# shao-lab/MotifScan

Measured on AMD Instinct MI355X. Metric: scanned bp*motifs per second (region_bp x n_motifs), both strands, p=1e-4 cutoffs, higher is better.
Workload: dtype f64 (every hit decision and score, as in the reference) behind an fp6 x fp4 one-hot matrix-core pre-filter (exact f32 accumulate)

## Files before the change

### motifscan_amd/csrc/ms_order.hip

```cpp
#include <algorithm>

#include "ms_device.h"

namespace ms {

namespace {

constexpr int kOrderThreads = 256;
constexpr int kOrderTile = 1024;
constexpr int kOrderExt = 256;
constexpr int kOrderWin = kOrderTile + kOrderExt;
constexpr int kOverflowBlocks = 256;

struct OrderRun {
    int64_t start;
    uint64_t prev;
};

struct OrderOut {
    int64_t *seq_idx;
    int64_t *pos;
    int8_t *strand;
    double *score;
    int64_t *motif_first;
    unsigned long long *region_counts;
    int rbits, pbits;
    int32_t P;
};

__device__ __forceinline__ bool decode_hit(const OrderOut &O, int64_t g, int64_t n, uint64_t k, double v, bool has_prev, uint64_t pk,
                                           uint32_t *motif_out) {
    const int ms = O.rbits + O.pbits + 1;
    const uint64_t pair = k >> (O.pbits + 1);
    const uint32_t motif = (uint32_t) (k >> ms);
    O.seq_idx[g] = (int64_t) (pair & ((1ULL << O.rbits) - 1ULL));
    O.pos[g] = (int64_t) ((k >> 1) & ((1ULL << O.pbits) - 1ULL));
    O.strand[g] = (int8_t) ((k & 1ULL) ? 2 : 1);
    O.score[g] = v;
    const uint32_t pm = has_prev ? (uint32_t) (pk >> ms) : 0u;
    if (!has_prev || pm != motif)
        for (int64_t q = has_prev ? (int64_t) pm + 1 : 0; q <= (int64_t) motif; q++) O.motif_first[q] = g;
    if (g == n - 1)
        for (int64_t q = (int64_t) motif + 1; q <= O.P; q++) O.motif_first[q] = n;
    *motif_out = motif;
    return !has_prev || (pk >> (O.pbits + 1)) != pair;
}

constexpr int kOrderMotifSlots = 8;
__device__ __forceinline__ void count_pairs(unsigned long long *region_counts, bool new_pair, uint32_t motif, unsigned int *lds, uint32_t m_base) {
    unsigned long long todo = __ballot(new_pair);
    while (todo) {
        const int leader = __ffsll((long long) todo) - 1;
        const uint32_t m = __shfl(motif, leader);
        const unsigned long long same = __ballot(new_pair && motif == m);
        if ((int) (threadIdx.x & 63) == leader) {
            if (lds && m - m_base < (uint32_t) kOrderMotifSlots) atomicAdd(&lds[m - m_base], (unsigned int) __popcll(same));
            else atomicAdd(&region_counts[m], (unsigned long long) __popcll(same));
        }
        todo &= ~same;
    }
}

__global__ void __launch_bounds__(kOrderThreads) order_finalize_kernel(const uint64_t *__restrict__ keys, int64_t n, const unsigned long long *__restrict__ n_dev,
                                                                      int L, int run_cap, OrderOut O, OrderRun *__restrict__ ovf,
                                                                      unsigned long long *__restrict__ ovf_n, uint64_t ovf_cap) {
    constexpr int kPer = kOrderWin / kOrderThreads, kSegs = kOrderWin / 64;
    __shared__ uint64_t K[kOrderWin];
    __shared__ uint64_t S[kOrderWin];
    __shared__ double V[kOrderWin];
    __shared__ uint8_t D[kOrderWin];
    __shared__ int seg_first[kSegs], seg_last[kSegs];
    __shared__ unsigned int rc[kOrderMotifSlots];
    if (n_dev) { const unsigned long long nd = *n_dev; if ((unsigned long long) n > nd) n = (int64_t) nd; }
    const int64_t s0 = (int64_t) blockIdx.x * kOrderTile;
    if (s0 >= n) return;
    const int tid = (int) threadIdx.x, lane = tid & 63, w = tid >> 6;
    const int wn = (int) std::min<int64_t>(kOrderWin, n - s0);
    const int tn = std::min(kOrderTile, wn);
    uint64_t kr[kPer];
    double vr[kPer];
#pragma unroll
    for (int k = 0; k < kPer; k++) {
        const int i = tid + kOrderThreads * k;
        kr[k] = i < wn ? keys[s0 + i] : ~0ULL;
        vr[k] = i < wn ? O.score[s0 + i] : 0.0;
        K[i] = kr[k];
        D[i] = 0;
    }
    if (tid < kOrderMotifSlots) rc[tid] = 0;
    const uint64_t prevk = s0 > 0 ? keys[s0 - 1] : 0ULL;
    __syncthreads();
    unsigned long long msk[kPer];
#pragma unroll
    for (int k = 0; k < kPer; k++) {
        const int i = tid + kOrderThreads * k;
        const bool start = i < wn && (i == 0 ? (s0 == 0 || (prevk >> L) != (kr[k] >> L)) : (K[i - 1] >> L) != (kr[k] >> L));
        msk[k] = __ballot(start);
        if (lane == 0) {
            const int seg = w + (kOrderThreads / 64) * k;
            seg_first[seg] = msk[k] ? seg * 64 + __ffsll((long long) msk[k]) - 1 : kOrderWin;
            seg_last[seg] = msk[k] ? seg * 64 + 63 - __clzll((long long) msk[k]) : -1;
        }
    }
    __syncthreads();
    int lo = kOrderWin, hi = wn;
    for (int q = 0; q < kSegs; q++) lo = std::min(lo, seg_first[q]);
    if (tn == kOrderTile)
        for (int q = kOrderTile / 64; q < kSegs; q++) hi = std::min(hi, seg_first[q]);
    if (lo >= tn) return;
    const bool closed = hi < wn || s0 + wn == n;
    const int ms = O.rbits + O.pbits + 1;
    const uint32_t m_base = (uint32_t) (K[lo] >> ms);
    const unsigned long long le = lane == 63 ? ~0ULL : (2ULL << lane) - 1ULL;
#pragma unroll
    for (int k = 0; k < kPer; k++) {
        const int i = tid + kOrderThreads * k, seg = w + (kOrderThreads / 64) * k;
        if (i < lo || i >= hi) continue;
        int a = -1, b = wn;
        if (msk[k] & le) a = seg * 64 + 63 - __clzll((long long) (msk[k] & le));
        else for (int q = seg - 1; q >= 0 && a < 0; q--) a = seg_last[q];
        if (msk[k] & ~le) b = seg * 64 + __ffsll((long long) (msk[k] & ~le)) - 1;
        else for (int q = seg + 1; q < kSegs && b == wn; q++) b = std::min(wn, seg_first[q]);
        if ((b == hi && !closed) || b - a > run_cap) {
            if (i == a) {
                const unsigned long long e = atomicAdd(ovf_n, 1ULL);
                if (e < ovf_cap) ovf[e] = OrderRun{s0 + a, a > 0 ? K[a - 1] : prevk};
            }
            continue;
        }
        int rank = 0;
        for (int j = a; j < b; j++) rank += K[j] < kr[k] ? 1 : 0;
        S[a + rank] = kr[k];
        V[a + rank] = vr[k];
        D[a + rank] = 1;
    }
    __syncthreads();
#pragma unroll
    for (int k = 0; k < kPer; k++) {
        const int j = tid + kOrderThreads * k;
        bool new_pair = false;
        uint32_t motif = 0;
        if (j >= lo && j < hi && D[j]) {
            const bool run_start = (msk[k] >> lane) & 1ULL;
            const uint64_t pk = run_start ? (j == 0 ? prevk : K[j - 1]) : S[j - 1];
            new_pair = decode_hit(O, s0 + j, n, S[j], V[j], s0 + j > 0, pk, &motif);
        }
        count_pairs(O.region_counts, new_pair, motif, rc, m_base);
    }
    __syncthreads();
    if (tid < kOrderMotifSlots && rc[tid]) atomicAdd(&O.region_counts[m_base + tid], (unsigned long long) rc[tid]);
}

__global__ void __launch_bounds__(kOrderThreads) order_overflow_kernel(uint64_t *keys, uint64_t *tmp_keys, double *tmp_vals,
                                                                      int64_t n, const unsigned long long *__restrict__ n_dev, int L, OrderOut O,
                                                                      const OrderRun *__restrict__ ovf, const unsigned long long *__restrict__ ovf_n,
                                                                      uint64_t ovf_cap) {
    __shared__ uint32_t base[256];
    __shared__ uint32_t wcnt[kOrderThreads / 64][256];
    __shared__ int64_t s_end;
    if (n_dev) { const unsigned long long nd = *n_dev; if ((unsigned long long) n > nd) n = (int64_t) nd; }
    const unsigned long long cnt = std::min<unsigned long long>(*ovf_n, ovf_cap);
    const int tid = (int) threadIdx.x, lane = tid & 63, w = tid >> 6;
    const unsigned long long lt = (1ULL << lane) - 1ULL;
    for (unsigned long long e = blockIdx.x; e < cnt; e += gridDim.x) {
        const int64_t s = ovf[e].start;
        const uint64_t prev = ovf[e].prev;
        const uint64_t h = keys[s] >> L;
        if (tid == 0) s_end = n;
        __syncthreads();
        for (int64_t c = s + 1; c < n; c += kOrderThreads) {
            const int64_t j = c + tid;
            if (j < n && (keys[j] >> L) != h) atomicMin((unsigned long long *) &s_end, (unsigned long long) j);
            __syncthreads();
            if (s_end < n) break;
            __syncthreads();
        }
        const int64_t b = s_end;
        uint64_t *sk = keys, *dk = tmp_keys;
        double *sv = O.score, *dv = tmp_vals;
        for (int shift = 0; shift < L; shift += 8) {
            base[tid] = 0;
            for (int q = 0; q < kOrderThreads / 64; q++) wcnt[q][tid] = 0;
            __syncthreads();
            for (int64_t j = s + tid; j < b; j += kOrderThreads) atomicAdd(&base[(uint32_t) (sk[j] >> shift) & 255u], 1u);
            __syncthreads();
            if (tid == 0) {
                uint32_t acc = 0;
                for (int d = 0; d < 256; d++) { const uint32_t c = base[d]; base[d] = acc; acc += c; }
            }
            __syncthreads();
            for (int64_t c = s; c < b; c += kOrderThreads) {
                const int64_t j = c + tid;
                const bool live = j < b;
                const uint64_t k = live ? sk[j] : 0ULL;
                const double v = live ? sv[j] : 0.0;
                const uint32_t d = (uint32_t) (k >> shift) & 255u;
                unsigned long long peers = __ballot(live);
#pragma unroll
                for (int bit = 0; bit < 8; bit++) {
                    const unsigned long long m = __ballot((d >> bit) & 1u);
                    peers &= ((d >> bit) & 1u) ? m : ~m;
                }
                if (live && (peers >> lane) == 1ULL) wcnt[w][d] = (uint32_t) __popcll(peers);
                __syncthreads();
                if (live) {
                    uint32_t off = base[d] + (uint32_t) __popcll(peers & lt);
                    for (int q = 0; q < w; q++) off += wcnt[q][d];
                    dk[s + off] = k;
                    dv[s + off] = v;
                }
                __syncthreads();
                uint32_t add = 0;
                for (int q = 0; q < kOrderThreads / 64; q++) { add += wcnt[q][tid]; wcnt[q][tid] = 0; }
                base[tid] += add;
                __syncthreads();
            }
            uint64_t *tk = sk; sk = dk; dk = tk;
            double *tv = sv; sv = dv; dv = tv;
        }
        for (int64_t c = s; c < b; c += kOrderThreads) {
            const int64_t j = c + tid;
            bool new_pair = false;
            uint32_t motif = 0;
            if (j < b) new_pair = decode_hit(O, j, n, sk[j], sv[j], j > 0, j == s ? prev : sk[j - 1], &motif);
            count_pairs(O.region_counts, new_pair, motif, nullptr, 0);
        }
        __syncthreads();
    }
}

}

size_t order_overflow_bytes(size_t n, int run_cap) {
    const size_t min_len = (size_t) std::min(std::max(run_cap, 1), kOrderExt) + 1;
    return (n / min_len + 1) * sizeof(OrderRun);
}

int launch_order_finalize(uint64_t *keys, double *score, int64_t n, const unsigned long long *n_dev, int L, int rbits, int pbits, int32_t P,
                          int64_t *seq_idx, int64_t *pos, int8_t *strand, int64_t *motif_first, unsigned long long *region_counts,
                          uint64_t *tmp_keys, double *tmp_vals, void *ovf_buf, size_t ovf_bytes, unsigned long long *ovf_n, int run_cap,
                          hipStream_t st) {
    if (n == 0 || n_dev) {
        MS_HIP(hipMemsetAsync(motif_first, 0, ((size_t) P + 1) * sizeof(int64_t), st));
        if (n == 0) return MS_OK;
    }
    run_cap = std::max(run_cap, 1);
    OrderOut O;
    O.seq_idx = seq_idx; O.pos = pos; O.strand = strand; O.score = score; O.motif_first = motif_first; O.region_counts = region_counts;
    O.rbits = rbits; O.pbits = pbits; O.P = P;
    OrderRun *ovf = static_cast<OrderRun *>(ovf_buf);
    const uint64_t ovf_cap = ovf_bytes / sizeof(OrderRun);
    hipLaunchKernelGGL(order_finalize_kernel, dim3((unsigned) ((n + kOrderTile - 1) / kOrderTile)), dim3(kOrderThreads), 0, st, keys, n, n_dev,
                       L, run_cap, O, ovf, ovf_n, ovf_cap);
    MS_HIP(hipGetLastError());
    if (L < 63 && (1ULL << L) > (unsigned long long) std::min(run_cap, kOrderExt)) {
        hipLaunchKernelGGL(order_overflow_kernel, dim3(kOverflowBlocks), dim3(kOrderThreads), 0, st, keys, tmp_keys, tmp_vals, n, n_dev, L, O,
                           ovf, ovf_n, ovf_cap);
        MS_HIP(hipGetLastError());
    }
    return MS_OK;
}


__global__ void __launch_bounds__(256) fill_tail_kernel(uint64_t *__restrict__ keys, const unsigned long long *__restrict__ n_dev, uint64_t cap) {
    const unsigned long long n = *n_dev < cap ? *n_dev : cap;
    for (unsigned long long i = n + (unsigned long long) blockIdx.x * blockDim.x + threadIdx.x; i < cap; i += (unsigned long long) gridDim.x * blockDim.x)
        keys[i] = ~0ULL;
}

__global__ void __launch_bounds__(256) sort_fixup_kernel(uint64_t *__restrict__ keys, double *__restrict__ vals, int64_t n, const unsigned long long *__restrict__ n_dev) {
    if (n_dev) { const unsigned long long nd = *n_dev; if ((unsigned long long) n > nd) n = (int64_t) nd; }
    const int64_t i0 = ((int64_t) blockIdx.x * blockDim.x + threadIdx.x) * 4;
    if (i0 >= n) return;
    uint64_t k[4] = {0, 0, 0, 0};
    uint64_t hi[6];
    hi[0] = i0 > 0 ? keys[i0 - 1] >> kSortLowBits : ~0ULL;
    if (i0 + 4 <= n) {
        const ulonglong2 a = *reinterpret_cast<const ulonglong2 *>(keys + i0), b = *reinterpret_cast<const ulonglong2 *>(keys + i0 + 2);
        k[0] = a.x; k[1] = a.y; k[2] = b.x; k[3] = b.y;
    } else {
        for (int q = 0; q < 4; q++) k[q] = i0 + q < n ? keys[i0 + q] : ~0ULL;
    }
#pragma unroll
    for (int q = 0; q < 4; q++) hi[1 + q] = i0 + q < n ? k[q] >> kSortLowBits : ~0ULL;
    hi[5] = i0 + 4 < n ? keys[i0 + 4] >> kSortLowBits : ~0ULL;
#pragma unroll
    for (int q = 0; q < 4; q++) {
        const int64_t i = i0 + q;
        if (i + 1 >= n || hi[1 + q] == hi[q] || hi[1 + q] != hi[2 + q]) continue;
        if (q < 3 && hi[3 + q] != hi[1 + q]) {
            if (k[q] > k[q + 1]) {
                keys[i] = k[q + 1];
                keys[i + 1] = k[q];
                const double v0 = vals[i], v1 = vals[i + 1];
                vals[i] = v1;
                vals[i + 1] = v0;
            }
            continue;
        }
        const uint64_t h = hi[1 + q];
        int64_t len = 2;
        while (i + len < n && len < ((int64_t) 1 << kSortLowBits) && (keys[i + len] >> kSortLowBits) == h) len++;
        for (int64_t a = 1; a < len; a++) {
            const uint64_t ka = keys[i + a];
            const double va = vals[i + a];
            int64_t b = a;
            while (b > 0 && keys[i + b - 1] > ka) { keys[i + b] = keys[i + b - 1]; vals[i + b] = vals[i + b - 1]; b--; }
            keys[i + b] = ka;
            vals[i + b] = va;
        }
    }
}

int launch_sort_fixup(uint64_t *keys, double *vals, int64_t n, const unsigned long long *n_dev, hipStream_t st) {
    if (n == 0) return MS_OK;
    hipLaunchKernelGGL(sort_fixup_kernel, dim3((unsigned) ((n + 1023) / 1024)), dim3(256), 0, st, keys, vals, n, n_dev);
    MS_HIP(hipGetLastError());
    return MS_OK;
}

__global__ void __launch_bounds__(kOrderBuckets) bucket_plan_kernel(const BucketWeights bw, double mu, unsigned long long n_pred, unsigned long long need,
                                                                    unsigned long long cap_max, unsigned long long *__restrict__ tab) {
    __shared__ unsigned long long sum[kOrderBuckets];
    const int b = (int) threadIdx.x;
    const unsigned long long w = bw.w[b];
    unsigned long long cb = 0;
    if (w) {
        const double e = mu * (double) w / (double) bw.total;
        cb = (unsigned long long) ceil(e + 6.0 * __dsqrt_rn(e + 1.0)) + 1ULL;
        const unsigned long long extra = n_pred > need ? n_pred - need : 0ULL;
        cb += (unsigned long long) floor((double) extra * (double) w / (double) bw.total);
    }
    if (cb > cap_max) cb = cap_max;
    sum[b] = cb;
    __syncthreads();
    for (int d = 1; d < kOrderBuckets; d <<= 1) {
        const unsigned long long v = b >= d ? sum[b - d] : 0ULL;
        __syncthreads();
        sum[b] += v;
        __syncthreads();
    }
    const unsigned long long at = sum[b] - cb, base = at < n_pred ? at : n_pred;
    tab[b] = base;
    tab[kOrderBuckets + b] = cb < n_pred - base ? cb : n_pred - base;
    tab[2 * kOrderBuckets + b] = 0ULL;
    if (b == kOrderBuckets - 1) tab[3 * kOrderBuckets] = sum[b] < n_pred ? sum[b] : n_pred;
}

__global__ void __launch_bounds__(256) fill_tail_buckets_kernel(uint64_t *__restrict__ keys, const unsigned long long *__restrict__ tab, uint64_t n_pred,
                                                                unsigned long long *__restrict__ n_hits, unsigned long long *__restrict__ overflow) {
    const unsigned int b = blockIdx.y;
    unsigned long long lo, hi;
    if (b < (unsigned int) kOrderBuckets) {
        const unsigned long long base = tab[b], cap = tab[kOrderBuckets + b], fill = tab[2 * kOrderBuckets + b];
        lo = base + (fill < cap ? fill : cap);
        hi = base + cap;
        if (fill > cap && blockIdx.x == 0 && threadIdx.x == 0) *overflow = 1ULL;
    } else {
        lo = tab[3 * kOrderBuckets];
        hi = n_pred;
        if (blockIdx.x == 0) {
            __shared__ unsigned long long part[256];
            unsigned long long v = 0;
            for (int q = (int) threadIdx.x; q < kOrderBuckets; q += 256) {
                const unsigned long long cap = tab[kOrderBuckets + q], fill = tab[2 * kOrderBuckets + q];
                v += fill < cap ? fill : cap;
            }
            part[threadIdx.x] = v;
            __syncthreads();
            for (int d = 128; d > 0; d >>= 1) {
                if ((int) threadIdx.x < d) part[threadIdx.x] += part[threadIdx.x + d];
                __syncthreads();
            }
            if (threadIdx.x == 0) *n_hits = part[0];
        }
    }
    if (hi > n_pred) hi = n_pred;
    for (unsigned long long i = lo + (unsigned long long) blockIdx.x * blockDim.x + threadIdx.x; i < hi; i += (unsigned long long) gridDim.x * blockDim.x)
        keys[i] = ~0ULL;
}

int launch_bucket_plan(const BucketWeights &bw, double mu, unsigned long long n_pred, unsigned long long need, unsigned long long cap_max,
                       unsigned long long *tab, hipStream_t st) {
    hipLaunchKernelGGL(bucket_plan_kernel, dim3(1), dim3(kOrderBuckets), 0, st, bw, mu, n_pred, need, cap_max, tab);
    MS_HIP(hipGetLastError());
    return MS_OK;
}

int launch_fill_tail_buckets(uint64_t *keys, const unsigned long long *tab, uint64_t n_pred, unsigned long long *n_hits, unsigned long long *overflow,
                             hipStream_t st) {
    hipLaunchKernelGGL(fill_tail_buckets_kernel, dim3(16, kOrderBuckets + 1), dim3(256), 0, st, keys, tab, n_pred, n_hits, overflow);
    MS_HIP(hipGetLastError());
    return MS_OK;
}

int launch_fill_tail(uint64_t *keys, const unsigned long long *n_dev, uint64_t cap, hipStream_t st) {
    if (cap == 0) return MS_OK;
    hipLaunchKernelGGL(fill_tail_kernel, dim3(256), dim3(256), 0, st, keys, n_dev, cap);
    MS_HIP(hipGetLastError());
    return MS_OK;
}

__global__ void __launch_bounds__(256) finalize_kernel(const uint64_t *__restrict__ keys, int64_t n, const unsigned long long *__restrict__ n_dev,
                                                       int gbits, int32_t P, const DevSeq S,
                                                       int64_t *__restrict__ seq_idx, int64_t *__restrict__ pos,
// ... 128 lines not shown
```

### motifscan_amd/csrc/ms_fp64.hip

```cpp
#include "ms_device.h"

namespace ms {

__device__ __forceinline__ int64_t hit_coord(const HitOut &H, const DevSeq &S, int64_t r, int64_t g) {
    return H.pbits ? (int64_t) (((uint64_t) r << H.pbits) | (uint64_t) (g - S.offsets[r])) : g;
}

__device__ __forceinline__ void emit_hit(const HitOut &H, uint32_t motif, int64_t g, uint32_t sbit, double score) {
    const unsigned long long i = atomicAdd(H.n_hits, 1ULL);
    if (i < H.cap) {
        H.keys[i] = ((uint64_t) motif << (H.gbits + 1)) | ((uint64_t) g << 1) | sbit;
        H.vals[i] = score;
    }
}

__device__ __forceinline__ void test_and_emit(const HitOut &H, const DevPwm &Pw, uint32_t motif, int64_t g,
                                              double fwd, double rev, int strand_mask) {
    const double floor_ = Pw.raw_floor[motif];
    const bool try_f = (strand_mask & 1) && !(fwd < floor_);
    const bool try_r = (strand_mask & 2) && !(rev < floor_);
    if (!try_f && !try_r) return;
    const double max_raw = Pw.max_raw[motif];
    const double cutoff = Pw.cutoff[motif];
    const double s_f = try_f ? fwd / max_raw : 0.0, s_r = try_r ? rev / max_raw : 0.0;
// ... 89 lines not shown
    {
        const double2 *__restrict__ tab = Pw.tab2 + Pw.tab_off[p];
        for (int i = threadIdx.x; i < W * 4; i += 256) tab_lds[i] = tab[i];
        if (threadIdx.x == 0) tab_lds[W * 4] = make_double2(0.0, 0.0);
    }
    __syncthreads();
    const uint32_t zero = (uint32_t) W * 4u;
    for (int it = 0; it < kExactIter; it++) {
        const int64_t g = ((int64_t) blockIdx.x * kExactIter + it) * 256 + threadIdx.x;
        if (g >= S.n_bases) break;
        const int64_t r = find_region(S, g);
        if (g + W > S.offsets[r + 1]) continue;
        double fwd = 0.0, rev = 0.0;
        for (int c0 = 0; c0 < W; c0 += 32) {
            const uint64_t cw = code_window(S.codes, g + c0);
            const int n = (W - c0) < 32 ? (W - c0) : 32;
            const uint32_t skip = n_window(S.nmask, g + c0) | ~low_mask(n);
            for (int c1 = 0; c1 < n; c1 += 8) {
                double2 t[8];
#pragma unroll
                for (int k = 0; k < 8; k++) {
                    const int c = c1 + k;
                    const uint32_t idx = (uint32_t) (c0 + c) * 4u + ((uint32_t) (cw >> (2 * c)) & 3u);
                    t[k] = tab_lds[((skip >> c) & 1u) ? zero : idx];
                }
#pragma unroll
                for (int k = 0; k < 8; k++) { fwd += t[k].x; rev += t[k].y; }
            }
        }
        test_and_emit(H, Pw, (uint32_t) p, hit_coord(H, S, r, g), fwd, rev, strand_mask);
    }
}

constexpr int kRescoreU = 4;

__global__ void __launch_bounds__(256) rescore_kernel(const DevSeq S, const DevPwm Pw, const uint64_t *__restrict__ cand,
                                                      const unsigned long long *__restrict__ n_cand, uint64_t n_static, uint64_t cand_cap,
                                                      const FieldMeta *__restrict__ field_meta, int strand_mask,
                                                      const HitOut H) {
    __shared__ HitStage st;
    if (threadIdx.x == 0) st.n = 0;
    __syncthreads();
    unsigned long long n = n_static + *n_cand;
    if (n > cand_cap) n = cand_cap;
    constexpr int U = kRescoreU;
    const bool both = strand_mask == 3;
    const unsigned long long per_sub = (unsigned long long) gridDim.x * blockDim.x;
    const unsigned long long per_round = per_sub * U;
    const unsigned long long rounds = (n + per_round - 1) / per_round;
    const int4 *__restrict__ meta4 = reinterpret_cast<const int4 *>(field_meta);
    for (unsigned long long rd = 0; rd < rounds; rd++) {
        const unsigned long long i0 = rd * per_round + (unsigned long long) blockIdx.x * blockDim.x + threadIdx.x;
        uint64_t c[U];
        bool live[U];
#pragma unroll
        for (int u = 0; u < U; u++) {
            live[u] = i0 + u * per_sub < n;
            c[u] = live[u] ? cand[i0 + u * per_sub] : 0;
        }
        int64_t g[U];
        int4 bi[U];
        uint64_t cw[U];
        uint32_t nw[U], flags[U];
        int32_t group[U];
        int4 fm[U];
#pragma unroll
        for (int u = 0; u < U; u++) {
            g[u] = (int64_t) (c[u] >> 30);
            group[u] = (int32_t) ((c[u] >> 16) & 0x3FFFu);
            const uint32_t f = (uint32_t) c[u] & 0xFFFFu;
            flags[u] = both ? (f | (f >> 1)) & 0x5555u : f;
            bi[u] = S.blkinfo[g[u] >> 6];
            cw[u] = code_window(S.codes, g[u]);
            nw[u] = n_window(S.nmask, g[u]);
            fm[u] = flags[u] ? meta4[group[u] * kGroupFields + (__ffs((int) flags[u]) - 1)] : make_int4(-1, 0, 0, 0);
        }
        int64_t r[U], beg[U], end[U];
#pragma unroll
        for (int u = 0; u < U; u++) {
            const int64_t base = g[u] & ~(int64_t) 63;
            int64_t lo = bi[u].x, o0 = base + bi[u].y, o1 = base + bi[u].z, o2 = base + bi[u].w;
            if (bi[u].x < 0) {
                lo = S.blk2reg[g[u] >> 6];
                o0 = S.offsets[lo]; o1 = S.offsets[lo + 1];
                o2 = lo + 2 <= S.R ? S.offsets[lo + 2] : o1;
            }
            if (g[u] < o1) { r[u] = lo; beg[u] = o0; end[u] = o1; }
            else if (g[u] < o2) { r[u] = lo + 1; beg[u] = o1; end[u] = o2; }
            else { r[u] = find_region(S, g[u]); beg[u] = S.offsets[r[u]]; end[u] = S.offsets[r[u] + 1]; }
        }
#pragma unroll
        for (int u = 0; u < U; u++) {
            if (!live[u]) continue;
            const int64_t gk = H.pbits ? (int64_t) (((uint64_t) r[u] << H.pbits) | (uint64_t) (g[u] - beg[u])) : g[u];
            bool first = true;
            while (flags[u]) {
                const int field = __ffs((int) flags[u]) - 1;
                flags[u] &= flags[u] - 1u;
                int4 f4 = fm[u];
                if (!first) f4 = meta4[group[u] * kGroupFields + field];
                first = false;
                const int32_t m = f4.x;
                const int w = f4.y;
                if (m < 0) continue;
                if (g[u] + w > end[u]) continue;
                double fwd, rev;
                if (w <= 32 && Pw.tab32) score_window32(Pw.tab2, (uint32_t) f4.z, Pw.zero_bytes, w, cw[u], nw[u], fwd, rev);
                else score_window(S, Pw.tab2 + Pw.tab_off[m], w, g[u], fwd, rev);
                test_and_stage(st, H, Pw, (uint32_t) m, gk, fwd, rev, strand_mask, __int_as_float(f4.w));
            }
        }
        __syncthreads();
        const bool full = st.n > (unsigned int) (kHitStage - 256 * 2 * U);
        __syncthreads();
        if (full) stage_flush(st, H);
    }
    stage_flush(st, H);
}

int launch_exact_all(const DevSeq &S, const DevPwm &Pw, const int32_t *motifs, int32_t n_motifs, int strand_mask,
                     const HitOut &H, hipStream_t st, int max_width) {
    if (S.n_bases == 0 || n_motifs == 0) return MS_OK;
    const bool tiled = max_width >= 1 && max_width <= kExactTileMaxW && !measure_env("MS_EXACT_UNTILED");
    const size_t lds = tiled ? ((size_t) max_width * 4 + 1) * sizeof(double2) : 0;
    if (tiled && lds > 48 * 1024)
        MS_HIP(hipFuncSetAttribute(reinterpret_cast<const void *>(exact_tiled_kernel), hipFuncAttributeMaxDynamicSharedMemorySize, (int) lds));
    for (int32_t m0 = 0; m0 < n_motifs; m0 += 32768) {
        const int32_t n = n_motifs - m0 < 32768 ? n_motifs - m0 : 32768;
        if (tiled) {
            dim3 grid((unsigned) ((S.n_bases + 256 * kExactIter - 1) / (256 * kExactIter)), (unsigned) n);
            hipLaunchKernelGGL(exact_tiled_kernel, grid, dim3(256), lds, st, S, Pw, motifs + m0, strand_mask, H);
        } else {
            dim3 grid((unsigned) ((S.n_bases + 255) / 256), (unsigned) n);
            hipLaunchKernelGGL(exact_all_kernel, grid, dim3(256), 0, st, S, Pw, motifs + m0, strand_mask, H);
        }
        MS_HIP(hipGetLastError());
    }
    return MS_OK;
}

int launch_rescore(const DevSeq &S, const DevPwm &Pw, const uint64_t *cand, const unsigned long long *n_cand, uint64_t n_static,
                   uint64_t cand_cap, const FieldMeta *field_meta, int strand_mask, const HitOut &H, int n_blocks,
                   hipStream_t st) {
    hipLaunchKernelGGL(rescore_kernel, dim3((unsigned) n_blocks), dim3(256), 0, st, S, Pw, cand, n_cand, n_static, cand_cap,
                       field_meta, strand_mask, H);
    MS_HIP(hipGetLastError());
    return MS_OK;
}

constexpr int kRwThreads = 1024;
constexpr int kRwPerThread = 4;
constexpr int kRwChunk = kRwThreads * kRwPerThread;
constexpr int kRwBins = 4096;
typedef HitStageN<2048> RwStage;
struct RwStageBk : RwStage {
    unsigned int cnt[kOrderBuckets], room[kOrderBuckets];
    unsigned long long lo[kOrderBuckets];
};

__device__ __forceinline__ void stage_flush(RwStageBk &st, const BucketHitOut &H) {
    constexpr int kPer = RwStageBk::kCap / kRwThreads;
    static_assert(kPer * kRwThreads == RwStageBk::kCap && kOrderBuckets <= kRwThreads, "stage_flush: one pass of the block over the stage");
    __syncthreads();
    const unsigned int n = st.n < (unsigned int) RwStageBk::kCap ? st.n : (unsigned int) RwStageBk::kCap;
    if (threadIdx.x < (unsigned int) kOrderBuckets) st.cnt[threadIdx.x] = 0;
    __syncthreads();
    uint32_t bk[kPer], rank[kPer];
#pragma unroll
    for (int k = 0; k < kPer; k++) {
        const unsigned int i = threadIdx.x + (unsigned int) (k * kRwThreads);
        bk[k] = i < n ? (uint32_t) (st.keys[i] >> H.B.shift) & 255u : 0u;
        rank[k] = i < n ? atomicAdd(&st.cnt[bk[k]], 1u) : 0u;
    }
    __syncthreads();
    if (threadIdx.x < (unsigned int) kOrderBuckets && st.cnt[threadIdx.x] > 0) {
        const unsigned int b = threadIdx.x, c = st.cnt[b];
        const unsigned long long f = atomicAdd(&H.B.fill[b], (unsigned long long) c), cap = H.B.cap[b];
        const unsigned long long left = f < cap ? cap - f : 0ULL;
        st.lo[b] = H.B.base[b] + f;
        st.room[b] = left < (unsigned long long) c ? (unsigned int) left : c;
        if (left < (unsigned long long) c) *H.B.overflow = 1ULL;
    }
    __syncthreads();
#pragma unroll
    for (int k = 0; k < kPer; k++) {
        const unsigned int i = threadIdx.x + (unsigned int) (k * kRwThreads);
        if (i < n && rank[k] < st.room[bk[k]]) {
            const unsigned long long at = st.lo[bk[k]] + rank[k];
            if (at < H.cap) { H.keys[at] = st.keys[i]; H.vals[at] = st.vals[i]; }
        }
    }
    __syncthreads();
    if (threadIdx.x == 0) st.n = 0;
    __syncthreads();
}

template <class HO, class ST>
__global__ void __launch_bounds__(kRwThreads) rescore_carry_kernel(const DevSeq S, const DevPwm Pw, const uint64_t *__restrict__ cand,
                                                                   const unsigned long long *__restrict__ n_cand, uint64_t n_static, uint64_t cand_cap,
                                                                   const FieldMeta *__restrict__ field_meta, int strand_mask, const HO H) {
    extern __shared__ uint4 rw_lds4[];
    uint64_t *s_cw = reinterpret_cast<uint64_t *>(rw_lds4);
    uint64_t *s_gk = s_cw + kRwChunk;
    uint32_t *s_nw = reinterpret_cast<uint32_t *>(s_gk + kRwChunk);
    uint32_t *s_gf = s_nw + kRwChunk;
    uint32_t *bins = s_gf + kRwChunk;
    uint32_t *wave_tot = bins + kRwBins;
    ST &st = *reinterpret_cast<ST *>(wave_tot + 32);
    if (threadIdx.x == 0) st.n = 0;
    unsigned long long n = n_static + *n_cand;
    if (n > cand_cap) n = cand_cap;
    const bool both = strand_mask == 3;
    const int4 *__restrict__ meta4 = reinterpret_cast<const int4 *>(field_meta);
    const uint32_t lane = threadIdx.x & 63u, wave = threadIdx.x >> 6;
    const uint64_t pmask = H.pbits ? ((1ULL << H.pbits) - 1ULL) : 0ULL;
    const unsigned long long n_chunks = (n + kRwChunk - 1) / kRwChunk;
    for (unsigned long long ch = blockIdx.x; ch < n_chunks; ch += gridDim.x) {
        for (uint32_t i = threadIdx.x; i < (uint32_t) kRwBins; i += kRwThreads) bins[i] = 0;
        __syncthreads();
        {
            uint64_t cw[kRwPerThread], gk[kRwPerThread];
            uint32_t nw[kRwPerThread], gf[kRwPerThread], key[kRwPerThread], rank[kRwPerThread];
            int64_t g[kRwPerThread];
            int4 bi[kRwPerThread];
#pragma unroll
            for (int k = 0; k < kRwPerThread; k++) {
                const unsigned long long i = ch * kRwChunk + (unsigned long long) k * kRwThreads + threadIdx.x;
                const uint64_t rec = i < n ? cand[i] : 0ULL;
                g[k] = (int64_t) (rec >> 30);
                gf[k] = (uint32_t) rec & 0x3FFFFFFFu;
                if (!(gf[k] & 0xFFFFu)) { gf[k] = 0; g[k] = 0; }
                bi[k] = S.blkinfo[g[k] >> 6];
                cw[k] = code_window(S.codes, g[k]);
                nw[k] = n_window(S.nmask, g[k]);
            }
#pragma unroll
            for (int k = 0; k < kRwPerThread; k++) {
                const int64_t base = g[k] & ~(int64_t) 63;
                int64_t lo = bi[k].x, o0 = base + bi[k].y, o1 = base + bi[k].z, o2 = base + bi[k].w, r, beg, end;
                if (bi[k].x < 0) {
                    lo = S.blk2reg[g[k] >> 6];
                    o0 = S.offsets[lo]; o1 = S.offsets[lo + 1];
                    o2 = lo + 2 <= S.R ? S.offsets[lo + 2] : o1;
                }
                if (g[k] < o1) { r = lo; beg = o0; end = o1; }
                else if (g[k] < o2) { r = lo + 1; beg = o1; end = o2; }
                else { r = find_region(S, g[k]); beg = S.offsets[r]; end = S.offsets[r + 1]; }
                const uint64_t coord = H.pbits ? (((uint64_t) r << H.pbits) | (uint64_t) (g[k] - beg)) : (uint64_t) g[k];
                const int64_t room = end - g[k];
                gk[k] = (coord << 8) | (uint64_t) (room > 255 ? 255 : (room < 0 ? 0 : room));
                const uint32_t f = gf[k] & 0xFFFFu;
                const uint32_t fl = both ? (f | (f >> 1)) & 0x5555u : f;
                key[k] = fl ? (((gf[k] >> 16) << 4) | (uint32_t) (__ffs((int) fl) - 1)) & (uint32_t) (kRwBins - 1) : (uint32_t) (kRwBins - 1);
            }
#pragma unroll
            for (int k = 0; k < kRwPerThread; k++) rank[k] = atomicAdd(&bins[key[k]], 1u);
            __syncthreads();
            {
                const uint32_t b0 = bins[4 * threadIdx.x], b1 = bins[4 * threadIdx.x + 1], b2 = bins[4 * threadIdx.x + 2], b3 = bins[4 * threadIdx.x + 3];
                const uint32_t tot = b0 + b1 + b2 + b3;
                uint32_t v = tot;
#pragma unroll
                for (int d = 1; d < 64; d <<= 1) {
                    const uint32_t o = __shfl_up(v, d);
                    if ((int) lane >= d) v += o;
                }
                if (lane == 63u) wave_tot[wave] = v;
                __syncthreads();
                uint32_t base = 0;
                for (uint32_t w = 0; w < wave; w++) base += wave_tot[w];
                const uint32_t excl = base + v - tot;
                bins[4 * threadIdx.x] = excl;
                bins[4 * threadIdx.x + 1] = excl + b0;
                bins[4 * threadIdx.x + 2] = excl + b0 + b1;
                bins[4 * threadIdx.x + 3] = excl + b0 + b1 + b2;
            }
            __syncthreads();
#pragma unroll
            for (int k = 0; k < kRwPerThread; k++) {
                const uint32_t at = bins[key[k]] + rank[k];
                s_cw[at] = cw[k]; s_gk[at] = gk[k]; s_nw[at] = nw[k]; s_gf[at] = gf[k];
            }
        }
        __syncthreads();
        for (int round = 0; round < 2; round++) {
#pragma unroll
            for (int u = 0; u < 2; u++) {
                const uint32_t at = (uint32_t) (round * 2 + u) * kRwThreads + threadIdx.x;
                const uint32_t gfu = s_gf[at];
                const uint32_t f = gfu & 0xFFFFu;
                uint32_t flags = both ? (f | (f >> 1)) & 0x5555u : f;
                if (!flags) continue;
                const uint64_t cwu = s_cw[at], gku = s_gk[at];
                const uint32_t nwu = s_nw[at];
                const int32_t group = (int32_t) (gfu >> 16);
                const int room = (int) (gku & 0xFFu);
                const int64_t coord = (int64_t) (gku >> 8);
                while (flags) {
                    const int field = __ffs((int) flags) - 1;
                    flags &= flags - 1u;
                    const int4 f4 = meta4[group * kGroupFields + field];
                    const int32_t m = f4.x;
                    const int w = f4.y;
                    if (m < 0) continue;
                    if (w > room) continue;
                    double fwd, rev;
                    if (w <= 32 && Pw.tab32) score_window32(Pw.tab2, (uint32_t) f4.z, Pw.zero_bytes, w, cwu, nwu, fwd, rev);
                    else {
                        const int64_t gpos = H.pbits ? S.offsets[coord >> H.pbits] + (int64_t) ((uint64_t) coord & pmask) : coord;
                        score_window(S, Pw.tab2 + Pw.tab_off[m], w, gpos, fwd, rev);
                    }
                    test_and_stage(st, H, Pw, (uint32_t) m, coord, fwd, rev, strand_mask, __int_as_float(f4.w));
                }
            }
            stage_flush(st, H);
        }
    }
}

template <class ST>
static size_t rescore_carry_lds_bytes() { return (size_t) kRwChunk * 24 + (size_t) kRwBins * 4 + 32 * 4 + sizeof(ST) + 64; }
int rescore_carry_set_lds() {
    MS_HIP(hipFuncSetAttribute(reinterpret_cast<const void *>(rescore_carry_kernel<HitOut, RwStage>), hipFuncAttributeMaxDynamicSharedMemorySize,
                               (int) rescore_carry_lds_bytes<RwStage>()));
    MS_HIP(hipFuncSetAttribute(reinterpret_cast<const void *>(rescore_carry_kernel<BucketHitOut, RwStageBk>), hipFuncAttributeMaxDynamicSharedMemorySize,
                               (int) rescore_carry_lds_bytes<RwStageBk>()));
    return MS_OK;
}
int launch_rescore_carry(const DevSeq &S, const DevPwm &Pw, const uint64_t *cand, const unsigned long long *n_cand, uint64_t n_static,
                         uint64_t cand_cap, const FieldMeta *field_meta, int strand_mask, const HitOut &H, int n_blocks, hipStream_t st) {
    hipLaunchKernelGGL((rescore_carry_kernel<HitOut, RwStage>), dim3((unsigned) n_blocks), dim3(kRwThreads), rescore_carry_lds_bytes<RwStage>(), st, S, Pw,
                       cand, n_cand, n_static, cand_cap, field_meta, strand_mask, H);
    MS_HIP(hipGetLastError());
    return MS_OK;
}
int launch_rescore_carry_bucketed(const DevSeq &S, const DevPwm &Pw, const uint64_t *cand, const unsigned long long *n_cand, uint64_t n_static,
                                  uint64_t cand_cap, const FieldMeta *field_meta, int strand_mask, const HitOut &H, const BucketOut &B, int n_blocks,
                                  hipStream_t st) {
    BucketHitOut HB;
    static_cast<HitOut &>(HB) = H;
    HB.B = B;
    hipLaunchKernelGGL((rescore_carry_kernel<BucketHitOut, RwStageBk>), dim3((unsigned) n_blocks), dim3(kRwThreads), rescore_carry_lds_bytes<RwStageBk>(), st,
                       S, Pw, cand, n_cand, n_static, cand_cap, field_meta, strand_mask, HB);
    MS_HIP(hipGetLastError());
    return MS_OK;
}

}
```

Baseline: 14800 billion.

## Fuse rank scatter and hit decode in finalize kernel, enlarge tile

The order-finalize kernel no longer scatters each key into shared sorted buffers (S, V, D) and then decodes in a second pass after a barrier. Each thread now computes its rank in the run and its sorted predecessor, which is the largest smaller key in the run, in the same scan, then calls decode_hit directly. This removes three shared arrays and one __syncthreads. The tile also grows from 1024 to 1792 with 512 threads per block. That cuts block count, but it also shrinks overlap redundancy and changes run-boundary overflow behaviour. Equal keys within a run would get the same rank, which could change semantics if duplicates exist.

Result: no change. 14910 billion, median of 6 (+0.8%).

```diff
diff --git a/motifscan_amd/csrc/ms_order.hip b/motifscan_amd/csrc/ms_order.hip
--- a/motifscan_amd/csrc/ms_order.hip
+++ b/motifscan_amd/csrc/ms_order.hip
@@ -7,9 +7,10 @@
 namespace {
 
 constexpr int kOrderThreads = 256;
-constexpr int kOrderTile = 1024;
+constexpr int kOrderTile = 1792;
 constexpr int kOrderExt = 256;
 constexpr int kOrderWin = kOrderTile + kOrderExt;
+constexpr int kFinalizeThreads = 512;
 constexpr int kOverflowBlocks = 256;
 
 struct OrderRun {
@@ -61,14 +62,12 @@
     }
 }
 
-__global__ void __launch_bounds__(kOrderThreads) order_finalize_kernel(const uint64_t *__restrict__ keys, int64_t n, const unsigned long long *__restrict__ n_dev,
+__global__ void __launch_bounds__(kFinalizeThreads) order_finalize_kernel(const uint64_t *__restrict__ keys, int64_t n, const unsigned long long *__restrict__ n_dev,
                                                                       int L, int run_cap, OrderOut O, OrderRun *__restrict__ ovf,
                                                                       unsigned long long *__restrict__ ovf_n, uint64_t ovf_cap) {
-    constexpr int kPer = kOrderWin / kOrderThreads, kSegs = kOrderWin / 64;
+    constexpr int kPer = kOrderWin / kFinalizeThreads, kSegs = kOrderWin / 64;
+    static_assert(kOrderWin % kFinalizeThreads == 0 && kFinalizeThreads % 64 == 0 && kOrderTile % 64 == 0, "whole segments per wave");
     __shared__ uint64_t K[kOrderWin];
-    __shared__ uint64_t S[kOrderWin];
-    __shared__ double V[kOrderWin];
-    __shared__ uint8_t D[kOrderWin];
     __shared__ int seg_first[kSegs], seg_last[kSegs];
     __shared__ unsigned int rc[kOrderMotifSlots];
     if (n_dev) { const unsigned long long nd = *n_dev; if ((unsigned long long) n > nd) n = (int64_t) nd; }
@@ -81,11 +80,10 @@
     double vr[kPer];
 #pragma unroll
     for (int k = 0; k < kPer; k++) {
-        const int i = tid + kOrderThreads * k;
+        const int i = tid + kFinalizeThreads * k;
         kr[k] = i < wn ? keys[s0 + i] : ~0ULL;
         vr[k] = i < wn ? O.score[s0 + i] : 0.0;
         K[i] = kr[k];
-        D[i] = 0;
     }
     if (tid < kOrderMotifSlots) rc[tid] = 0;
     const uint64_t prevk = s0 > 0 ? keys[s0 - 1] : 0ULL;
@@ -93,11 +91,11 @@
     unsigned long long msk[kPer];
 #pragma unroll
     for (int k = 0; k < kPer; k++) {
-        const int i = tid + kOrderThreads * k;
+        const int i = tid + kFinalizeThreads * k;
         const bool start = i < wn && (i == 0 ? (s0 == 0 || (prevk >> L) != (kr[k] >> L)) : (K[i - 1] >> L) != (kr[k] >> L));
         msk[k] = __ballot(start);
         if (lane == 0) {
-            const int seg = w + (kOrderThreads / 64) * k;
+            const int seg = w + (kFinalizeThreads / 64) * k;
             seg_first[seg] = msk[k] ? seg * 64 + __ffsll((long long) msk[k]) - 1 : kOrderWin;
             seg_last[seg] = msk[k] ? seg * 64 + 63 - __clzll((long long) msk[k]) : -1;
         }
@@ -114,36 +112,31 @@
     const unsigned long long le = lane == 63 ? ~0ULL : (2ULL << lane) - 1ULL;
 #pragma unroll
     for (int k = 0; k < kPer; k++) {
-        const int i = tid + kOrderThreads * k, seg = w + (kOrderThreads / 64) * k;
-        if (i < lo || i >= hi) continue;
-        int a = -1, b = wn;
-        if (msk[k] & le) a = seg * 64 + 63 - __clzll((long long) (msk[k] & le));
-        else for (int q = seg - 1; q >= 0 && a < 0; q--) a = seg_last[q];
-        if (msk[k] & ~le) b = seg * 64 + __ffsll((long long) (msk[k] & ~le)) - 1;
-        else for (int q = seg + 1; q < kSegs && b == wn; q++) b = std::min(wn, seg_first[q]);
-        if ((b == hi && !closed) || b - a > run_cap) {
-            if (i == a) {
-                const unsigned long long e = atomicAdd(ovf_n, 1ULL);
-                if (e < ovf_cap) ovf[e] = OrderRun{s0 + a, a > 0 ? K[a - 1] : prevk};
-            }
-            continue;
-        }
-        int rank = 0;
-        for (int j = a; j < b; j++) rank += K[j] < kr[k] ? 1 : 0;
-        S[a + rank] = kr[k];
-        V[a + rank] = vr[k];
-        D[a + rank] = 1;
-    }
-    __syncthreads();
-#pragma unroll
-    for (int k = 0; k < kPer; k++) {
-        const int j = tid + kOrderThreads * k;
+        const int i = tid + kFinalizeThreads * k, seg = w + (kFinalizeThreads / 64) * k;
         bool new_pair = false;
         uint32_t motif = 0;
-        if (j >= lo && j < hi && D[j]) {
-            const bool run_start = (msk[k] >> lane) & 1ULL;
-            const uint64_t pk = run_start ? (j == 0 ? prevk : K[j - 1]) : S[j - 1];
-            new_pair = decode_hit(O, s0 + j, n, S[j], V[j], s0 + j > 0, pk, &motif);
+        if (i >= lo && i < hi) {
+            int a = -1, b = wn;
+            if (msk[k] & le) a = seg * 64 + 63 - __clzll((long long) (msk[k] & le));
+            else for (int q = seg - 1; q >= 0 && a < 0; q--) a = seg_last[q];
+            if (msk[k] & ~le) b = seg * 64 + __ffsll((long long) (msk[k] & ~le)) - 1;
+            else for (int q = seg + 1; q < kSegs && b == wn; q++) b = std::min(wn, seg_first[q]);
+            if ((b == hi && !closed) || b - a > run_cap) {
+                if (i == a) {
+                    const unsigned long long e = atomicAdd(ovf_n, 1ULL);
+                    if (e < ovf_cap) ovf[e] = OrderRun{s0 + a, a > 0 ? K[a - 1] : prevk};
+                }
+            } else {
+                int rank = 0;
+                uint64_t pk = 0;
+                for (int j = a; j < b; j++) {
+                    const uint64_t kj = K[j];
+                    if (kj < kr[k]) { rank++; pk = std::max(pk, kj); }
+                }
+                if (rank == 0) pk = a > 0 ? K[a - 1] : prevk;
+                const int64_t g = s0 + a + rank;
+                new_pair = decode_hit(O, g, n, kr[k], vr[k], g > 0, pk, &motif);
+            }
         }
         count_pairs(O.region_counts, new_pair, motif, rc, m_base);
     }
@@ -250,7 +243,7 @@
     O.rbits = rbits; O.pbits = pbits; O.P = P;
     OrderRun *ovf = static_cast<OrderRun *>(ovf_buf);
     const uint64_t ovf_cap = ovf_bytes / sizeof(OrderRun);
-    hipLaunchKernelGGL(order_finalize_kernel, dim3((unsigned) ((n + kOrderTile - 1) / kOrderTile)), dim3(kOrderThreads), 0, st, keys, n, n_dev,
+    hipLaunchKernelGGL(order_finalize_kernel, dim3((unsigned) ((n + kOrderTile - 1) / kOrderTile)), dim3(kFinalizeThreads), 0, st, keys, n, n_dev,
                        L, run_cap, O, ovf, ovf_n, ovf_cap);
     MS_HIP(hipGetLastError());
     if (L < 63 && (1ULL << L) > (unsigned long long) std::min(run_cap, kOrderExt)) {
```

## Stage rescore hits in per-candidate LDS slots with spill area, flush once per chunk

Applied to the files above, without the earlier changes.

The rescore-carry kernel no longer appends every hit to a shared LDS stage via atomics and flushes it twice per chunk. Each candidate's first hit is written in place into its own LDS slot, reusing the code-window and key arrays. Extra hits go to a wave-aggregated spill area, and everything is flushed once per chunk with a block prefix scan and a single global atomic. This cuts LDS atomic contention and flush barriers, at the cost of a smaller spill buffer that falls back to per-hit global atomics when it overflows.

New measurement: 14320 billion before, 14380 billion after (median of 6 runs). About the same (+0.4%).

```diff
diff --git a/motifscan_amd/csrc/ms_fp64.hip b/motifscan_amd/csrc/ms_fp64.hip
--- a/motifscan_amd/csrc/ms_fp64.hip
+++ b/motifscan_amd/csrc/ms_fp64.hip
@@ -265,47 +265,146 @@
 constexpr int kRwPerThread = 4;
 constexpr int kRwChunk = kRwThreads * kRwPerThread;
 constexpr int kRwBins = 4096;
-typedef HitStageN<2048> RwStage;
-struct RwStageBk : RwStage {
+constexpr int kRwSpill = 1024;
+struct RwSpill {
+    uint64_t keys[kRwSpill];
+    double vals[kRwSpill];
+    unsigned int n;
+    unsigned long long base;
+};
+struct RwSpillBk : RwSpill {
     unsigned int cnt[kOrderBuckets], room[kOrderBuckets];
     unsigned long long lo[kOrderBuckets];
 };
 
-__device__ __forceinline__ void stage_flush(RwStageBk &st, const BucketHitOut &H) {
-    constexpr int kPer = RwStageBk::kCap / kRwThreads;
-    static_assert(kPer * kRwThreads == RwStageBk::kCap && kOrderBuckets <= kRwThreads, "stage_flush: one pass of the block over the stage");
-    __syncthreads();
-    const unsigned int n = st.n < (unsigned int) RwStageBk::kCap ? st.n : (unsigned int) RwStageBk::kCap;
-    if (threadIdx.x < (unsigned int) kOrderBuckets) st.cnt[threadIdx.x] = 0;
-    __syncthreads();
-    uint32_t bk[kPer], rank[kPer];
+template <class HO>
+__device__ __forceinline__ void spill_hit(RwSpill &sp, const HO &H, uint32_t motif, int64_t g, uint32_t sbit, double score) {
+    const uint64_t act = __ballot(1);
+    const uint32_t r = __builtin_amdgcn_mbcnt_hi((uint32_t) (act >> 32), __builtin_amdgcn_mbcnt_lo((uint32_t) act, 0u));
+    uint32_t first = 0;
+    if (r == 0) first = atomicAdd(&sp.n, (unsigned int) __popcll(act));
+    const uint32_t i = (uint32_t) __builtin_amdgcn_readfirstlane((int) first) + r;
+    if (i < (uint32_t) kRwSpill) {
+        sp.keys[i] = ((uint64_t) motif << (H.gbits + 1)) | ((uint64_t) g << 1) | sbit;
+        sp.vals[i] = score;
+    } else {
+        emit_hit(H, motif, g, sbit, score);
+    }
+}
+
+template <class HO>
+__device__ __forceinline__ void test_and_place(uint64_t &slot_key, uint64_t &slot_val, uint32_t &mine, RwSpill &sp, const HO &H, const DevPwm &Pw,
+                                               uint32_t motif, int64_t g, double fwd, double rev, int strand_mask, float floor32) {
+    const double floor_ = (double) floor32;
+    const bool try_f = (strand_mask & 1) && !(fwd < floor_);
+    const bool try_r = (strand_mask & 2) && !(rev < floor_);
+    if (!try_f && !try_r) return;
+    const double2 mc = *reinterpret_cast<const double2 *>(Pw.thresh + 4 * (size_t) motif);
+    const double max_raw = mc.x, cutoff = mc.y;
+#pragma unroll
+    for (uint32_t sbit = 0; sbit < 2; sbit++) {
+        if (!(sbit ? try_r : try_f)) continue;
+        const double s = (sbit ? rev : fwd) / max_raw;
+        if (!(s - cutoff >= -1e-10)) continue;
+        if (!mine) {
+            slot_key = ((uint64_t) motif << (H.gbits + 1)) | ((uint64_t) g << 1) | sbit;
+            slot_val = (uint64_t) __double_as_longlong(s);
+            mine = 1u;
+        } else {
+            spill_hit(sp, H, motif, g, sbit, s);
+        }
+    }
+}
+
+__device__ __forceinline__ void chunk_flush(const uint64_t *keys, const uint64_t *vals, const uint32_t *taken, uint32_t *wave_tot, RwSpill &sp,
+                                            const HitOut &H) {
+    const uint32_t lane = threadIdx.x & 63u, wave = threadIdx.x >> 6;
+    __syncthreads();
+    const uint4 t4 = *reinterpret_cast<const uint4 *>(taken + 4 * threadIdx.x);
+    const uint32_t tot = t4.x + t4.y + t4.z + t4.w;
+    uint32_t v = tot;
+#pragma unroll
+    for (int d = 1; d < 64; d <<= 1) {
+        const uint32_t o = __shfl_up(v, d);
+        if ((int) lane >= d) v += o;
+    }
+    if (lane == 63u) wave_tot[wave] = v;
+    __syncthreads();
+    uint32_t before = 0, in_place = 0;
+    for (uint32_t w = 0; w < (uint32_t) (kRwThreads / 64); w++) {
+        const uint32_t t = wave_tot[w];
+        if (w < wave) before += t;
+        in_place += t;
+    }
+    const uint32_t n_sp = sp.n < (unsigned int) kRwSpill ? sp.n : (unsigned int) kRwSpill;
+    if (threadIdx.x == 0 && in_place + n_sp > 0) sp.base = atomicAdd(H.n_hits, (unsigned long long) (in_place + n_sp));
+    __syncthreads();
+    const unsigned long long base = sp.base;
+    unsigned long long at = base + (before + v - tot);
+    const uint32_t t[4] = {t4.x, t4.y, t4.z, t4.w};
+#pragma unroll
+    for (int j = 0; j < 4; j++) {
+        if (!t[j]) continue;
+        if (at < H.cap) { H.keys[at] = keys[4 * threadIdx.x + j]; H.vals[at] = __longlong_as_double((long long) vals[4 * threadIdx.x + j]); }
+        at++;
+    }
+    for (uint32_t i = threadIdx.x; i < n_sp; i += kRwThreads) {
+        const unsigned long long to = base + in_place + i;
+        if (to < H.cap) { H.keys[to] = sp.keys[i]; H.vals[to] = sp.vals[i]; }
+    }
+}
+
+__device__ __forceinline__ void chunk_flush(const uint64_t *keys, const uint64_t *vals, const uint32_t *taken, uint32_t *, RwSpillBk &sp,
+                                            const BucketHitOut &H) {
+    constexpr int kPer = kRwSpill / kRwThreads;
+    static_assert(kPer * kRwThreads == kRwSpill && kOrderBuckets <= kRwThreads, "chunk_flush: one pass of the block over the spill area");
+    __syncthreads();
+    const uint4 t4 = *reinterpret_cast<const uint4 *>(taken + 4 * threadIdx.x);
+    const uint32_t t[4] = {t4.x, t4.y, t4.z, t4.w};
+    const uint32_t n_sp = sp.n < (unsigned int) kRwSpill ? sp.n : (unsigned int) kRwSpill;
+    uint32_t bk[4 + kPer], rank[4 + kPer];
+#pragma unroll
+    for (int j = 0; j < 4; j++) {
+        bk[j] = t[j] ? (uint32_t) (keys[4 * threadIdx.x + j] >> H.B.shift) & 255u : 0u;
+        rank[j] = t[j] ? atomicAdd(&sp.cnt[bk[j]], 1u) : 0u;
+    }
 #pragma unroll
     for (int k = 0; k < kPer; k++) {
         const unsigned int i = threadIdx.x + (unsigned int) (k * kRwThreads);
-        bk[k] = i < n ? (uint32_t) (st.keys[i] >> H.B.shift) & 255u : 0u;
-        rank[k] = i < n ? atomicAdd(&st.cnt[bk[k]], 1u) : 0u;
-    }
-    __syncthreads();
-    if (threadIdx.x < (unsigned int) kOrderBuckets && st.cnt[threadIdx.x] > 0) {
-        const unsigned int b = threadIdx.x, c = st.cnt[b];
+        bk[4 + k] = i < n_sp ? (uint32_t) (sp.keys[i] >> H.B.shift) & 255u : 0u;
+        rank[4 + k] = i < n_sp ? atomicAdd(&sp.cnt[bk[4 + k]], 1u) : 0u;
+    }
+    __syncthreads();
+    if (threadIdx.x < (unsigned int) kOrderBuckets && sp.cnt[threadIdx.x] > 0) {
+        const unsigned int b = threadIdx.x, c = sp.cnt[b];
         const unsigned long long f = atomicAdd(&H.B.fill[b], (unsigned long long) c), cap = H.B.cap[b];
         const unsigned long long left = f < cap ? cap - f : 0ULL;
-        st.lo[b] = H.B.base[b] + f;
-        st.room[b] = left < (unsigned long long) c ? (unsigned int) left : c;
+        sp.lo[b] = H.B.base[b] + f;
+        sp.room[b] = left < (unsigned long long) c ? (unsigned int) left : c;
         if (left < (unsigned long long) c) *H.B.overflow = 1ULL;
     }
     __syncthreads();
+#pragma unroll
+    for (int j = 0; j < 4; j++) {
+        if (t[j] && rank[j] < sp.room[bk[j]]) {
+            const unsigned long long at = sp.lo[bk[j]] + rank[j];
+            if (at < H.cap) { H.keys[at] = keys[4 * threadIdx.x + j]; H.vals[at] = __longlong_as_double((long long) vals[4 * threadIdx.x + j]); }
+        }
+    }
 #pragma unroll
     for (int k = 0; k < kPer; k++) {
         const unsigned int i = threadIdx.x + (unsigned int) (k * kRwThreads);
-        if (i < n && rank[k] < st.room[bk[k]]) {
-            const unsigned long long at = st.lo[bk[k]] + rank[k];
-            if (at < H.cap) { H.keys[at] = st.keys[i]; H.vals[at] = st.vals[i]; }
-        }
-    }
-    __syncthreads();
-    if (threadIdx.x == 0) st.n = 0;
-    __syncthreads();
+        if (i < n_sp && rank[4 + k] < sp.room[bk[4 + k]]) {
+            const unsigned long long at = sp.lo[bk[4 + k]] + rank[4 + k];
+            if (at < H.cap) { H.keys[at] = sp.keys[i]; H.vals[at] = sp.vals[i]; }
+        }
+    }
+}
+
+__device__ __forceinline__ void chunk_begin(RwSpill &sp) { if (threadIdx.x == 0) sp.n = 0; }
+__device__ __forceinline__ void chunk_begin(RwSpillBk &sp) {
+    if (threadIdx.x == 0) sp.n = 0;
+    if (threadIdx.x < (unsigned int) kOrderBuckets) sp.cnt[threadIdx.x] = 0;
 }
 
 template <class HO, class ST>
@@ -319,8 +418,7 @@
     uint32_t *s_gf = s_nw + kRwChunk;
     uint32_t *bins = s_gf + kRwChunk;
     uint32_t *wave_tot = bins + kRwBins;
-    ST &st = *reinterpret_cast<ST *>(wave_tot + 32);
-    if (threadIdx.x == 0) st.n = 0;
+    ST &sp = *reinterpret_cast<ST *>(wave_tot + 32);
     unsigned long long n = n_static + *n_cand;
     if (n > cand_cap) n = cand_cap;
     const bool both = strand_mask == 3;
@@ -331,6 +429,7 @@
     for (unsigned long long ch = blockIdx.x; ch < n_chunks; ch += gridDim.x) {
         for (uint32_t i = threadIdx.x; i < (uint32_t) kRwBins; i += kRwThreads) bins[i] = 0;
         __syncthreads();
+        chunk_begin(sp);
         {
             uint64_t cw[kRwPerThread], gk[kRwPerThread];
             uint32_t nw[kRwPerThread], gf[kRwPerThread], key[kRwPerThread], rank[kRwPerThread];
@@ -409,6 +508,7 @@
                 const int32_t group = (int32_t) (gfu >> 16);
                 const int room = (int) (gku & 0xFFu);
                 const int64_t coord = (int64_t) (gku >> 8);
+                uint32_t mine = 0;
                 while (flags) {
                     const int field = __ffs((int) flags) - 1;
                     flags &= flags - 1u;
@@ -423,26 +523,27 @@
                         const int64_t gpos = H.pbits ? S.offsets[coord >> H.pbits] + (int64_t) ((uint64_t) coord & pmask) : coord;
                         score_window(S, Pw.tab2 + Pw.tab_off[m], w, gpos, fwd, rev);
                     }
-                    test_and_stage(st, H, Pw, (uint32_t) m, coord, fwd, rev, strand_mask, __int_as_float(f4.w));
+                    test_and_place(s_cw[at], s_gk[at], mine, sp, H, Pw, (uint32_t) m, coord, fwd, rev, strand_mask, __int_as_float(f4.w));
                 }
-            }
-            stage_flush(st, H);
-        }
+                s_gf[at] = mine;
+            }
+        }
+        chunk_flush(s_cw, s_gk, s_gf, wave_tot, sp, H);
     }
 }
 
 template <class ST>
 static size_t rescore_carry_lds_bytes() { return (size_t) kRwChunk * 24 + (size_t) kRwBins * 4 + 32 * 4 + sizeof(ST) + 64; }
 int rescore_carry_set_lds() {
-    MS_HIP(hipFuncSetAttribute(reinterpret_cast<const void *>(rescore_carry_kernel<HitOut, RwStage>), hipFuncAttributeMaxDynamicSharedMemorySize,
-                               (int) rescore_carry_lds_bytes<RwStage>()));
-    MS_HIP(hipFuncSetAttribute(reinterpret_cast<const void *>(rescore_carry_kernel<BucketHitOut, RwStageBk>), hipFuncAttributeMaxDynamicSharedMemorySize,
-                               (int) rescore_carry_lds_bytes<RwStageBk>()));
+    MS_HIP(hipFuncSetAttribute(reinterpret_cast<const void *>(rescore_carry_kernel<HitOut, RwSpill>), hipFuncAttributeMaxDynamicSharedMemorySize,
+                               (int) rescore_carry_lds_bytes<RwSpill>()));
+    MS_HIP(hipFuncSetAttribute(reinterpret_cast<const void *>(rescore_carry_kernel<BucketHitOut, RwSpillBk>), hipFuncAttributeMaxDynamicSharedMemorySize,
+                               (int) rescore_carry_lds_bytes<RwSpillBk>()));
     return MS_OK;
 }
 int launch_rescore_carry(const DevSeq &S, const DevPwm &Pw, const uint64_t *cand, const unsigned long long *n_cand, uint64_t n_static,
                          uint64_t cand_cap, const FieldMeta *field_meta, int strand_mask, const HitOut &H, int n_blocks, hipStream_t st) {
-    hipLaunchKernelGGL((rescore_carry_kernel<HitOut, RwStage>), dim3((unsigned) n_blocks), dim3(kRwThreads), rescore_carry_lds_bytes<RwStage>(), st, S, Pw,
+    hipLaunchKernelGGL((rescore_carry_kernel<HitOut, RwSpill>), dim3((unsigned) n_blocks), dim3(kRwThreads), rescore_carry_lds_bytes<RwSpill>(), st, S, Pw,
                        cand, n_cand, n_static, cand_cap, field_meta, strand_mask, H);
     MS_HIP(hipGetLastError());
     return MS_OK;
@@ -453,7 +554,7 @@
     BucketHitOut HB;
     static_cast<HitOut &>(HB) = H;
     HB.B = B;
-    hipLaunchKernelGGL((rescore_carry_kernel<BucketHitOut, RwStageBk>), dim3((unsigned) n_blocks), dim3(kRwThreads), rescore_carry_lds_bytes<RwStageBk>(), st,
+    hipLaunchKernelGGL((rescore_carry_kernel<BucketHitOut, RwSpillBk>), dim3((unsigned) n_blocks), dim3(kRwThreads), rescore_carry_lds_bytes<RwSpillBk>(), st,
                        S, Pw, cand, n_cand, n_static, cand_cap, field_meta, strand_mask, HB);
     MS_HIP(hipGetLastError());
     return MS_OK;
```
